# ElesionKyrie/Extreme-Video-Compression-With-Prediction-Using-Pre-trainded-Diffusion-Models-

Measured on AMD Instinct MI355X. Metric: decoded frames/sec (128x128x30) at q3, higher is better.
Workload: dtype f32

## Files before the change

extreme-video-compression-with-prediction-using-pre-trainded-diffusion-models-_amd/csrc/conv_small.hip:

```cpp
#include <hip/hip_runtime.h>
#include <stdint.h>
#include <stdio.h>
#include "../../include/evc_hip.h"
#include "split_mfma.h"

namespace {

struct SmallK {
    const float* src0; const float* src1; int C0, C1;
    const float* coef_a; const float* coef_s; const unsigned* in_bound;
    const char* w;
    const float* w_hdr;
    const float* bias; const float* res; float out_scale;
    float* out; float* stats;
    int H, HW, Co, CoPad, nchunk;
    int MT, NT, linear;
};

__device__ __forceinline__ float small_silu(float v) { return v * __builtin_amdgcn_rcpf(1.0f + __expf(-v)); }

template <bool AFFINE>
__device__ __forceinline__ float4 small_transform(float4 v, const float4& a, const float4& s, bool ok) {
    if (AFFINE) {
        v.x = small_silu(v.x * a.x + s.x); v.y = small_silu(v.y * a.y + s.y);
// ... 213 lines not shown
                if (t == 3) {
                    stage_store((it & 1) ^ 1);
                    __builtin_amdgcn_sched_barrier(0);
                }
            }
        }
        __syncthreads();
    }

    float* const red = reinterpret_cast<float*>(smem);
    if (g > 0) {
        float* o = red + (size_t)((g - 1) * NW + wv) * (TM * 16 * 64) + lane;
#pragma unroll
        for (int i = 0; i < TM; ++i)
#pragma unroll
            for (int r = 0; r < 16; ++r) o[(i * 16 + r) * 64] = acc[i][r];
    }
    __syncthreads();
    if (g > 0) return;
#pragma unroll 1
    for (int gg = 1; gg < G; ++gg) {
        const float* o = red + (size_t)((gg - 1) * NW + wv) * (TM * 16 * 64) + lane;
#pragma unroll
        for (int i = 0; i < TM; ++i)
#pragma unroll
            for (int r = 0; r < 16; ++r) acc[i][r] += o[(i * 16 + r) * 64];
    }
    if (p.res) {
        if (p.stats) small_epilogue<true, true>(p, acc, m0, n0, wm, wn, l31, half);
        else small_epilogue<true, false>(p, acc, m0, n0, wm, wn, l31, half);
    } else {
        if (p.stats) small_epilogue<false, true>(p, acc, m0, n0, wm, wn, l31, half);
        else small_epilogue<false, false>(p, acc, m0, n0, wm, wn, l31, half);
    }
}


struct SmallVariant { int W, wm, wn, g; };
constexpr SmallVariant SMALL_VARIANTS[4] = {
    {8, 1, 1, 8},
    {8, 1, 2, 4},
    {16, 2, 1, 4},
    {16, 2, 2, 2},
};

struct SmallLaunch {
    int variant;
    bool affine;
    dim3 grid;
    int threads;
    SmallK k;
};

int small_resolve(const evc_small_conv_args* a, SmallLaunch& p) {
    if (!a || !a->src0 || !a->w_packed || !a->out) return EVC_EINVAL;
    if (a->B <= 0 || a->H <= 0 || a->W <= 0 || a->C0 <= 0 || a->C1 < 0 || a->Co <= 0) return EVC_EINVAL;
    if ((a->C1 > 0) != (a->src1 != nullptr)) return EVC_EINVAL;
    if ((a->coef_a != nullptr) != (a->coef_s != nullptr)) return EVC_EINVAL;
    if (a->arith != EVC_ARITH_F16X3) return EVC_EUNSUPPORTED;
    if (a->KH != 3 || a->KW != 3) return EVC_EUNSUPPORTED;
    if (a->H != a->W || (a->H != 8 && a->H != 16)) return EVC_EUNSUPPORTED;
    if (a->invariant || a->x2_w_packed) return EVC_EUNSUPPORTED;
    if (a->act_out != EVC_ACT_NONE) return EVC_EUNSUPPORTED;
    if (a->coef_a ? a->act_in != EVC_ACT_SILU : a->act_in != EVC_ACT_NONE) return EVC_EUNSUPPORTED;
    if (a->C0 % 16 != 0 || a->C1 % 16 != 0 || a->Co % 32 != 0) return EVC_EUNSUPPORTED;
    const long long HW = (long long)a->H * a->W, M = HW * a->B, Ct = (long long)a->C0 + a->C1;
// ... 42 lines not shown
    SmallLaunch p;
    return small_resolve(a, p) == EVC_OK ? 1 : 0;
}

extern "C" int evc_small_conv_plan_query(const evc_small_conv_args* a, evc_small_conv_plan* out) {
    SmallLaunch p;
    const int rc = !out ? EVC_EINVAL : small_resolve(a, p);
    if (rc != EVC_OK) return rc;
    const SmallVariant& sv = SMALL_VARIANTS[p.variant - 1];
    small_kernel_name(p, out->kernel, (int)sizeof(out->kernel));
    out->variant = p.variant; out->tile_m = 64 * sv.wm; out->tile_n = 32 * sv.wn; out->groups = sv.g;
    out->chunks = p.k.nchunk; out->rounds = (p.k.nchunk + sv.g - 1) / sv.g; out->stats_runs = p.k.HW / 64;
    return EVC_OK;
}

extern "C" int evc_small_conv_f32(const evc_small_conv_args* a, void* stream) {
    SmallLaunch p;
    const int rc = small_resolve(a, p);
    if (rc != EVC_OK) return rc;
    SmallK& k = p.k;
    k.src0 = a->src0; k.src1 = a->src1; k.coef_a = a->coef_a; k.coef_s = a->coef_s; k.in_bound = a->in_bound;
    k.w_hdr = a->w_packed;
    k.w = reinterpret_cast<const char*>(a->w_packed) + F16_HDR_BYTES;
    k.bias = a->bias; k.res = a->res; k.out_scale = a->out_scale; k.out = a->out; k.stats = a->stats_out;
    hipStream_t st = (hipStream_t)stream;
    switch (p.variant) {
        case 1: small_launch<1, 1, 8>(p, st); break;
        case 2: small_launch<1, 2, 4>(p, st); break;
        case 3: small_launch<2, 1, 4>(p, st); break;
        default: small_launch<2, 2, 2>(p, st); break;
    }
    return hipGetLastError() == hipSuccess ? EVC_OK : EVC_ELAUNCH;
}
```

extreme-video-compression-with-prediction-using-pre-trainded-diffusion-models-_amd/lib.py:

```python
import ctypes
import math
import os
from ctypes import POINTER, c_char_p, c_double, c_float, c_int, c_int32, c_longlong, c_uint, c_uint8, c_ulonglong, c_void_p

import numpy as np
import torch

HERE = os.path.dirname(os.path.abspath(__file__))
HIP_SO = os.path.join(HERE, "lib", "libevc_hip.so")
if os.environ.get("EVC_HIP_SO"):
    HIP_SO = os.path.abspath(os.environ["EVC_HIP_SO"])
RANS_SO = os.path.join(HERE, "lib", "libevc_rans.so")

ACT_NONE, ACT_SILU, ACT_RELU = 0, 1, 2
ARITH_F32, ARITH_BF16X6, ARITH_F16X3 = 0, 1, 2
_ARITH_NAMES = {"f32": ARITH_F32, "bf16x6": ARITH_BF16X6, "f16x3": ARITH_F16X3}
_ARITH_DTYPES = {ARITH_F32: torch.float32, ARITH_BF16X6: torch.bfloat16, ARITH_F16X3: torch.float16}


def _arith_policy():
    name = os.environ.get("EVC_CONV_ARITH", "f16x3").lower()
    if name not in _ARITH_NAMES:
        raise ValueError(f"EVC_CONV_ARITH must be one of {sorted(_ARITH_NAMES)}, got {name!r}")
    return _ARITH_NAMES[name]
# ... 28 lines not shown
                ("x2_src0", c_void_p), ("x2_src1", c_void_p), ("x2_C0", c_int), ("x2_C1", c_int), ("x2_ld0", c_int),
                ("x2_ld1", c_int), ("x2_w_packed", c_void_p), ("x2_bound", c_void_p), ("invariant", c_int)]


class ConvPlan(ctypes.Structure):
    _fields_ = [("kernel", ctypes.c_char * 96), ("tile_m", c_int), ("tile_n", c_int), ("splits", c_int),
                ("steps_per_split", c_int), ("cut_chunk", c_int), ("tail_tiles", c_int), ("tail_splits", c_int),
                ("stats_runs", c_int), ("fused_1x1", c_int)]


class NinArgs(ctypes.Structure):
    _fields_ = [("x", c_void_p), ("x1", c_void_p), ("Ci", c_int), ("Co", c_int), ("coef_a", c_void_p), ("coef_s", c_void_p),
                ("in_bound", c_void_p), ("w_packed", c_void_p), ("arith", c_int), ("bias", c_void_p), ("res", c_void_p),
                ("out_scale", c_float), ("act_out", c_int), ("out", c_void_p), ("stats_out", c_void_p),
                ("B", c_int), ("H", c_int), ("W", c_int), ("tile", c_int)]


class NinPlan(ctypes.Structure):
    _fields_ = [("kernel", ctypes.c_char * 64), ("tile_m", c_int), ("tile_n", c_int), ("stages", c_int), ("stats_runs", c_int)]


class SmallConvArgs(ctypes.Structure):
    _fields_ = [("src0", c_void_p), ("src1", c_void_p), ("C0", c_int), ("C1", c_int),
                ("coef_a", c_void_p), ("coef_s", c_void_p), ("act_in", c_int), ("in_bound", c_void_p),
                ("w_packed", c_void_p), ("arith", c_int), ("bias", c_void_p), ("res", c_void_p),
                ("out_scale", c_float), ("act_out", c_int), ("out", c_void_p), ("stats_out", c_void_p),
                ("B", c_int), ("H", c_int), ("W", c_int), ("Co", c_int), ("KH", c_int), ("KW", c_int),
                ("x2_w_packed", c_void_p), ("invariant", c_int), ("variant", c_int)]


class SmallConvPlan(ctypes.Structure):
    _fields_ = [("kernel", ctypes.c_char * 64), ("variant", c_int), ("tile_m", c_int), ("tile_n", c_int), ("groups", c_int),
                ("chunks", c_int), ("rounds", c_int), ("stats_runs", c_int)]


class AttentionPlan(ctypes.Structure):
    _fields_ = [("kernel", ctypes.c_char * 64), ("waves", c_int), ("kparts", c_int), ("tiles_per_part", c_int),
                ("kv_planes", c_int), ("merge", c_int), ("short_seq", c_int),
                ("lds_bytes", c_longlong), ("parts_bytes", c_longlong), ("ws_bytes", c_longlong)]


HIP_SYMBOLS = {
    "evc_version": (c_char_p, []),
    "evc_arch": (c_char_p, []),
    "evc_device_ok": (c_int, []),
    "evc_clock_probe": (c_int, [c_void_p, c_int, c_void_p, c_void_p]),
    "evc_im2col_nchw_f32": (c_int, [c_void_p, c_void_p] + [c_int] * 9 + [c_void_p, c_void_p, c_void_p]),
    "evc_maxpool3s2_nhwc_f32": (c_int, [c_void_p, c_void_p, c_int, c_int, c_int, c_int, c_void_p]),
    "evc_lpips_layer_f32": (c_int, [c_void_p, c_void_p, c_void_p, c_void_p, c_int, c_int, c_int, c_int, c_void_p]),
    "evc_maxpool2d_nhwc_f32": (c_int, [c_void_p, c_void_p] + [c_int] * 7 + [c_void_p]),
    "evc_lpips_map_f32": (c_int, [c_void_p, c_void_p, c_void_p, c_void_p, c_int, c_int, c_int, c_void_p]),
    "evc_lpips_map_mean_f32": (c_int, [c_void_p, c_void_p, c_int, c_int, c_int, c_void_p]),
    "evc_lpips_upsample_add_f32": (c_int, [c_void_p, c_void_p] + [c_int] * 6 + [c_void_p]),
    "evc_i3d_stem_im2col_f32": (c_int, [c_void_p, c_void_p] + [c_int] * 17 + [c_void_p]),
    "evc_maxpool3d_same_nthwc_f32": (c_int, [c_void_p, c_void_p] + [c_int] * 11 + [c_void_p]),
    "evc_i3d_head_f32": (c_int, [c_void_p] * 4 + [c_int] * 6 + [c_void_p]),
    "evc_upfirdn2d_f32": (c_int, [c_void_p, c_void_p, POINTER(c_float)] + [c_int] * 13 + [c_void_p]),
    "evc_upfirdn2d_nhwc_f32": (c_int, [c_void_p, c_void_p, POINTER(c_float)] + [c_int] * 10 +
                               [c_void_p, c_void_p, c_int, c_void_p]),
    "evc_pack_nchw_to_nhwc_f32": (c_int, [c_void_p, c_int, c_void_p, c_int, c_void_p, c_int, c_int, c_int, c_int,
                                          c_void_p]),
    "evc_nhwc_to_nchw_f32": (c_int, [c_void_p, c_int, c_void_p, c_int, c_int, c_int, c_int, c_void_p]),
    "evc_chan_stats_f32": (c_int, [c_void_p, c_void_p, c_int, c_int, c_int, c_int, c_void_p]),
    "evc_gn_coeffs_f32": (c_int, [c_void_p, c_int, c_int, c_void_p, c_int, c_int, c_int, c_int, c_int, c_float,
                                  c_int, c_void_p, c_void_p, c_void_p, c_int, c_void_p, c_void_p, c_void_p,
                                  c_void_p]),
# ... 25 lines not shown
    "evc_conv5x5s2_phase_weights_f32": (c_int, [c_void_p, c_void_p, c_int, c_int, c_int, c_void_p]),
    "evc_depth_to_space2_f32": (c_int, [c_void_p, c_int, c_int, c_void_p, c_int, c_int, c_int, c_int, c_void_p]),
    "evc_space_to_depth2_f32": (c_int, [c_void_p, c_int, c_int, c_void_p, c_int, c_int, c_int, c_int, c_int, c_void_p]),
    "evc_deconv5x5s2_workspace_bytes": (c_longlong, [c_int, c_int, c_int, c_int]),
    "evc_deconv5x5s2_f32": (c_int, [c_void_p, c_void_p, c_int, c_void_p, c_void_p, c_void_p] + [c_int] * 6 + [c_void_p]),
    "evc_conv5x5s2_workspace_bytes": (c_longlong, [c_int, c_int, c_int, c_int]),
    "evc_conv5x5s2_f32": (c_int, [c_void_p, c_int, c_void_p, c_int, c_void_p, c_void_p, c_void_p] + [c_int] * 6 + [c_void_p]),
    "evc_gdn_workspace_bytes": (c_longlong, [c_int, c_int, c_int, c_int]),
    "evc_gdn_f32": (c_int, [c_void_p, c_void_p, c_int, c_void_p, c_void_p, c_void_p, c_int, c_int, c_int, c_int, c_int,
                            c_int, c_void_p]),
    "evc_affine_act_nhwc_f32": (c_int, [c_void_p, c_void_p, c_void_p, c_void_p, c_int, c_int, c_int, c_int, c_int,
                                        c_int, c_void_p]),
    "evc_conv_co_pad": (c_int, [c_int]),
    "evc_conv_packed_floats": (c_longlong, [c_int, c_int, c_int, c_int]),
    "evc_conv_pack_weights_f32": (c_int, [c_void_p, c_void_p, c_int, c_int, c_int, c_int, c_void_p]),
    "evc_conv_packed_bytes": (c_longlong, [c_int, c_int, c_int, c_int, c_int]),
    "evc_conv_pack_weights": (c_int, [c_void_p, c_void_p, c_int, c_int, c_int, c_int, c_int, c_void_p]),
    "evc_conv_set_option": (c_int, [c_char_p, c_int]),
    "evc_spade_act_nhwc_f32": (c_int, [c_void_p, c_void_p, c_void_p, c_void_p, c_int, c_void_p, c_void_p, c_int, c_void_p,
                                       c_void_p, c_int, c_void_p, c_int, c_int, c_int, c_int, c_int, c_void_p]),
    "evc_conv_choose_splits": (c_int, [POINTER(ConvArgs)]),
    "evc_conv_kernel_name": (c_int, [POINTER(ConvArgs), c_char_p, c_int]),
    "evc_conv_fused_1x1_supported": (c_int, [POINTER(ConvArgs)]),
    "evc_conv_stats_splits": (c_int, [POINTER(ConvArgs)]),
    "evc_conv_workspace_bytes": (c_longlong, [POINTER(ConvArgs)]),
    "evc_conv2d_nhwc_f32": (c_int, [POINTER(ConvArgs), c_void_p, c_void_p]),
    "evc_conv2d_nhwc_profiled_f32": (c_int, [POINTER(ConvArgs), c_void_p, c_void_p, c_void_p, c_void_p]),
    "evc_nin_gemm_supported": (c_int, [POINTER(NinArgs)]),
    "evc_nin_gemm_plan_query": (c_int, [POINTER(NinArgs), POINTER(NinPlan)]),
    "evc_nin_gemm_f32": (c_int, [POINTER(NinArgs), c_void_p]),
    "evc_small_conv_supported": (c_int, [POINTER(SmallConvArgs)]),
    "evc_small_conv_plan_query": (c_int, [POINTER(SmallConvArgs), POINTER(SmallConvPlan)]),
    "evc_small_conv_f32": (c_int, [POINTER(SmallConvArgs), c_void_p]),
    "evc_attention_f32": (c_int, [c_void_p, c_void_p, c_void_p, c_int, c_void_p, c_int, c_int, c_int, c_int, c_int,
                                  c_float, c_void_p]),
    "evc_attention_workspace_bytes": (c_longlong, [c_int, c_int, c_int, c_int]),
    "evc_attention_set_option": (c_int, [c_char_p, c_int]),
    "evc_attention_plan_query": (c_int, [c_int, c_int, c_int, c_int, c_int, c_int, c_int, POINTER(AttentionPlan)]),
    "evc_attention_ws_f32": (c_int, [c_void_p, c_void_p, c_void_p, c_int, c_void_p, c_int, c_int, c_int, c_int, c_int,
                                     c_float, c_void_p, c_void_p]),
    "evc_frame_group_norm_f32": (c_int, [c_void_p] * 4 + [c_int] * 5 + [c_float, c_void_p]),
    "evc_frame_attention_f32": (c_int, [c_void_p, c_int, c_void_p, c_int] + [c_int] * 5 + [c_float, c_void_p]),
    "evc_frame_mix_f32": (c_int, [c_void_p] * 4 + [c_int] * 3 + [c_longlong, c_void_p]),
    "evc_frame_taps_f32": (c_int, [c_void_p, c_void_p] + [c_int] * 4 + [c_void_p]),
    "evc_ddpm_step_f32": (c_int, [c_void_p, c_void_p, c_void_p, c_longlong] + [c_float] * 5 + [c_int, c_void_p]),
    "evc_ddim_step_f32": (c_int, [c_void_p, c_void_p, c_longlong] + [c_float] * 4 + [c_int, c_void_p]),
    "evc_axpy_f32": (c_int, [c_void_p, c_void_p, c_void_p, c_longlong, c_float, c_void_p]),
    "evc_pndm_transfer_f32": (c_int, [c_void_p, c_void_p, c_void_p, c_longlong, c_float, c_float, c_float, c_int,
                                      c_void_p]),
    "evc_lincomb4_f32": (c_int, [c_void_p] * 5 + [c_longlong] + [c_float] * 4 + [c_void_p]),
    "evc_scale_clamp_f32": (c_int, [c_void_p, c_void_p, c_longlong, c_float, c_float, c_int, c_float, c_float,
                                    c_void_p]),
    "evc_gate_residual_f32": (c_int, [c_void_p, c_void_p, c_void_p, c_void_p, c_longlong, c_void_p]),
    "evc_elic_gather_params_f32": (c_int, [c_void_p] + [c_int] * 8 + [c_void_p, c_int, c_void_p, c_void_p,
                                                                       c_void_p]),
    "evc_elic_scatter_symbols_f32": (c_int, [c_void_p, c_void_p, c_void_p] + [c_int] * 7 + [c_void_p]),
    "evc_elic_quantize_f32": (c_int, [c_void_p, c_int, c_int, c_void_p] + [c_int] * 5 + [c_void_p, c_void_p]),
    "evc_elic_rate_pass_f32": (c_int, [c_void_p] + [c_int] * 4 + [c_void_p] + [c_int] * 6 + [c_void_p, c_void_p, c_void_p]),
    "evc_bottleneck_rate_f32": (c_int, [c_void_p] + [c_int] * 5 + [c_void_p] * 5),
    "evc_noise_normal_f32": (c_int, [c_void_p, c_void_p, c_int, c_longlong, c_ulonglong, c_uint, c_int, c_void_p]),
    "evc_yuv420_to_rgb": (c_int, [c_void_p] + [c_longlong] * 6 + [c_int] * 5 + [c_void_p, c_int, c_void_p]),
    "evc_rgb_to_yuv420": (c_int, [c_void_p, c_void_p] + [c_longlong] * 6 + [c_int] * 4 + [c_void_p, c_void_p]),
    "evc_resample_h_u8": (c_int, [c_void_p, c_int, c_int, c_int, c_longlong, c_longlong, c_void_p, c_void_p, c_int, c_int, c_void_p,
                                  c_void_p]),
    "evc_resample_v_u8": (c_int, [c_void_p, c_int, c_int, c_int, c_longlong, c_longlong, c_void_p, c_void_p, c_int, c_int, c_void_p,
                                  c_void_p]),
# ... 757 lines not shown
                chunks=out.chunks, rounds=out.rounds, stats_runs=out.stats_runs)


def small_conv(src0, w_packed, Co, bias=None, src1=None, coef=None, act_in=ACT_NONE, res=None, out_scale=1.0, in_bound=None,
               want_stats=False, out=None, variant=0):
    L = hip_lib()
    B, H, W, C0 = src0.shape
    C1 = 0 if src1 is None else src1.shape[-1]
    for t, c in ((src0, C0), (src1, C1), (res, Co)):
        assert t is None or (t.is_contiguous() and t.dtype == torch.float32 and t.shape == (B, H, W, c))
    if out is None:
        out = torch.empty((B, H, W, Co), device=src0.device, dtype=torch.float32)
    assert out.is_contiguous() and out.shape == (B, H, W, Co)
    ca, cs = coef if coef is not None else (None, None)
    assert ca is None or (ca.shape == (B, C0 + C1) and cs.shape == (B, C0 + C1) and ca.is_contiguous() and cs.is_contiguous())
    a = SmallConvArgs(src0=ptr(src0), src1=ptr(src1), C0=C0, C1=C1, coef_a=ptr(ca), coef_s=ptr(cs), act_in=act_in,
                      in_bound=_word(in_bound), w_packed=ptr(w_packed), arith=packed_arith(w_packed), bias=ptr(bias),
                      res=ptr(res), out_scale=float(out_scale), act_out=ACT_NONE, out=ptr(out), B=B, H=H, W=W, Co=Co, KH=3, KW=3,
                      variant=variant)
    plan = SmallConvPlan()
    _check(L.evc_small_conv_plan_query(ctypes.byref(a), ctypes.byref(plan)), "evc_small_conv_plan_query")
    stats = None
    if want_stats:
        stats = torch.empty((B, plan.stats_runs, Co, 2), device=src0.device, dtype=torch.float32)
        a.stats_out = ptr(stats)
    _check(L.evc_small_conv_f32(ctypes.byref(a), stream_ptr()), "evc_small_conv_f32")
    if SMALL_CONV_PROFILE is not None:
        SMALL_CONV_PROFILE.append(dict(kernel=plan.kernel.decode(), tile=(plan.tile_m, plan.tile_n), groups=plan.groups,
                                       shape=(B, H, W, C0 + C1, Co), C1=C1, coef=coef is not None, bound=in_bound is not None,
                                       res=res is not None, stats=bool(want_stats)))
    return (out, stats) if want_stats else out


def attention_set_option(name, value):
    if hip_lib(require_device=False).evc_attention_set_option(name.encode(), int(value)) != 0:
        raise EvcKernelError(f"unknown attention option {name!r}")


ATTN_PROFILE = None


def attention_plan(B, heads, N, D, with_bounds=False, have_ws=None, invariant=False):
    L = hip_lib(require_device=False)
    if have_ws is None:
        nbytes = (L.evc_attention_invariant_workspace_bytes if invariant else L.evc_attention_workspace_bytes)(B, heads, N, D)
        have_ws = nbytes > 0
    out = AttentionPlan()
    _check(L.evc_attention_plan_query(B, heads, N, D, int(bool(with_bounds)), int(bool(have_ws)), int(bool(invariant)),
                                      ctypes.byref(out)), "evc_attention_plan_query")
    return dict(kernel=out.kernel.decode(), waves=out.waves, kparts=out.kparts, tiles_per_part=out.tiles_per_part,
                kv_planes=bool(out.kv_planes), merge=bool(out.merge), short_seq=bool(out.short_seq),
                lds_bytes=out.lds_bytes, parts_bytes=out.parts_bytes, ws_bytes=out.ws_bytes)


def attention(qkv, C, heads, out=None, bounds=None, invariant=False, ws=None):
    L = hip_lib()
    B, N, ld = qkv.shape
    D = C // heads
    inv = bool(invariant)
    if out is None:
        out = torch.empty((B, N, C), device=qkv.device, dtype=torch.float32)
    ld_out = out.shape[-1]
    assert out.is_contiguous() and tuple(out.shape[:2]) == (B, N) and ld_out >= C
    base = qkv.data_ptr()
    nbytes = (L.evc_attention_invariant_workspace_bytes if inv else L.evc_attention_workspace_bytes)(B, heads, N, D)
    if ws is None:
# ... 542 lines not shown
```

extreme-video-compression-with-prediction-using-pre-trainded-diffusion-models-_amd/scorenet.py:

```python
import math
from types import SimpleNamespace

import numpy as np
import torch

from . import lib as L

FIR_K = np.outer([1, 3, 3, 1], [1, 3, 3, 1]).astype(np.float32)
FIR_K /= FIR_K.sum()
INV_SQRT2 = float(np.float32(1.0) / np.sqrt(np.float32(2.0)))


def num_groups(ch):
    g = min(ch // 4, 32)
    while ch % g != 0:
        g -= 1
    return g


def dims_from_config(config):
    m, d = config.model, config.data
    return SimpleNamespace(ngf=m.ngf, ch_mult=list(m.ch_mult), num_res_blocks=m.num_res_blocks,
                           attn_resolutions=list(m.attn_resolutions), n_head_channels=m.n_head_channels,
                           image_size=d.image_size, channels=d.channels, num_frames=d.num_frames,
# ... 170 lines not shown
        self.embed_dim = self._embed_dim()
        self.program = self._build_program()
        if self.SPADE:
            self.program[2]["cin"] = self.d.channels * self.d.num_frames
        self._wsrc = {}
        self._load(state_dict, prefix + "unet.all_modules.")
        self.sites = range_sites(self.program, self.cond_emb) if self.RANGE_SITES else []
        self.site_words = L.site_word_arena(len(self.sites), self.device)
        self._demoted = set()
        self._attn_f32 = set()
        self._unfused = set()
        self._site_of = {}
        self._set_site_args()
        self.demote_seconds = 0.0
        self._rows = {}
        self._row_tensors = {}
        self._table = torch.zeros((256, self.ss_total), device=self.device, dtype=torch.float32)
        self._n_rows = 0
        self.use_graphs = use_graphs
        self._graphs = {}
        self._f16_raw = L.bounded_arith() == L.ARITH_F16X3
        import os
        self.overlap_skip = os.environ.get("EVC_OVERLAP_SKIP", "1") != "0"
        self.fuse_skip = self._f16_raw and os.environ.get("EVC_FUSE_SKIP", "1") != "0"
        self._side_streams = {}
        self._bounds_by_stream = {}
        self._bounds = None
        self._bound_next = 0
        self._bound_batch = 1
        if demote:
            self.demote(demote)

    def _conv(self, *a, **kw):
        return self._conv_routed(*a, **kw) if self.small_conv else L.conv2d_nhwc(*a, invariant=self.batch_invariant, **kw)

    def _act(self, t, stats=None):
        return _Act(t, stats, invariant=self.batch_invariant)

    def _gn(self, *a, **kw):
        return L.gn_coeffs(*a, invariant=self.batch_invariant, **kw)

    def _mbound(self, *a, **kw):
        return L.moments_bound(*a, invariant=self.batch_invariant, **kw)

    def _attention(self, *a, **kw):
        return L.attention(*a, invariant=self.batch_invariant, **kw)

    def _fuse_ok(self, *a, **kw):
        return L.conv_fused_1x1_supported(*a, invariant=self.batch_invariant, **kw)

    def invariant_view(self):
        import copy
        if self.batch_invariant:
            return self
        if self.SPADE or self.ARCH != "unetmore" or self.noise_in_cond:
            raise NotImplementedError("batch_invariant is built for the concat-conditioned score network (ScoreNet) only")
        if self._demoted:
            raise ValueError("batch-invariant mode does not combine with demoted sites (range recovery)")
        v = copy.copy(self)
        v.batch_invariant = True
        v.taps = None
        v._rows, v._row_tensors = {}, {}
        v._table = torch.zeros_like(self._table)
        v._n_rows = 0
        v._graphs, v._side_streams, v._bounds_by_stream = {}, {}, {}
        v._bounds, v._bound_next = None, 0
        return v
# ... 267 lines not shown

    def _attn(self, i, m, x):
        e = self.w[i]
        B, H, W, C = x.t.shape
        hd = self.d.n_head_channels
        heads = 1 if C < hd else C // hd
        coef = self._gn([x.stats()], H * W, num_groups(C), 1e-6, mode=1, gamma=e["gamma"], beta=e["beta"],
                           site=self._site("attn_norm", i))
        qkvb = self._bound_slot(3)
        if qkvb is None:
            obound = None
            qkv = self._proj(x.t, e["wqkv"], 3 * C, e["bqkv"], coef=coef)
        else:
            qkv, qst = self._proj(x.t, e["wqkv"], 3 * C, e["bqkv"], coef=coef, want_stats=True)
            self._mbound(qst, 0, C, qkvb, site=self._site("attn_qkv", i))
            obound = _f16_only(e["wo"], qkvb.view(B, 3)[:, 2].contiguous() if self.batch_invariant else qkvb[2:3])
        o = self._attention(qkv.view(B, H * W, 3 * C), C, heads, bounds=None if i in self._attn_f32 else qkvb)
        return self._act(*self._proj(o.view(B, H, W, C), e["wo"], C, e["bo"], res=x.t, out_scale=INV_SQRT2, want_stats=True,
                                     in_bound=obound))

    nin_gemm = True

    def _proj(self, x, w, Co, bias, coef=None, res=None, out_scale=1.0, want_stats=False, in_bound=None):
        B, H, W, Ci = x.shape
        plain = not self.batch_invariant and not self.SPADE and self.ARCH == "unetmore"
        if self.nin_gemm and plain and L.packed_arith(w) == L.ARITH_F16X3 and \
                L.nin_gemm_supported(B, H, W, Ci, Co, coef=coef is not None, bound=in_bound is not None):
            return L.nin_gemm(x, w, Co, bias=bias, coef=coef, res=res, out_scale=out_scale, in_bound=in_bound,
                              want_stats=want_stats)
        return self._conv(x, w, Co, 1, 1, bias=bias, coef=coef, res=res, out_scale=out_scale, want_stats=want_stats,
                          in_bound=in_bound)

    small_conv = True

    def _conv_routed(self, src0, w, Co, KH, KW, src1=None, x2=None, out=None, act_out=L.ACT_NONE, splits=0, **kw):
        plain = not self.batch_invariant and not self.SPADE and self.ARCH == "unetmore"
        dense = torch.is_tensor(src0) and (src1 is None or torch.is_tensor(src1))
        if plain and dense and KH == 3 and KW == 3 and x2 is None and out is None and act_out == L.ACT_NONE and not splits \
                and L.packed_arith(w) == L.ARITH_F16X3:
            B, H, W, C0 = src0.shape
            if L.small_conv_supported(B, H, W, C0, 0 if src1 is None else src1.shape[-1], Co, coef=kw.get("coef") is not None,
                                      act_in=kw.get("act_in", L.ACT_NONE), bound=kw.get("in_bound") is not None):
                return L.small_conv(src0, w, Co, src1=src1, **kw)
        return L.conv2d_nhwc(src0, w, Co, KH, KW, src1=src1, x2=x2, out=out, act_out=act_out, splits=splits,
                             invariant=self.batch_invariant, **kw)

    @torch.no_grad()
    def forward_rows(self, x, rows, cond=None):
        if self.batch_invariant and self._demoted:
            raise ValueError("batch-invariant mode does not combine with demoted sites (range recovery)")
        return self._forward_rows(x, rows, cond)

    def _forward_rows(self, x, rows, cond=None):
        d = self.d
        prog = self.program
        B, _, H, W = x.shape
        self._bound_batch = B if self.batch_invariant else 1
        nb = 256 * self._bound_batch
        if self._f16_raw:
            if torch.cuda.is_current_stream_capturing():
                self._bounds = torch.empty(nb, device=self.device, dtype=torch.int32)
            else:
                key = torch.cuda.current_stream().cuda_stream
                self._bounds = self._bounds_by_stream.get(key)
                if self._bounds is None or self._bounds.numel() != nb:
                    self._bounds = self._bounds_by_stream[key] = torch.empty(nb, device=self.device, dtype=torch.int32)
            self._bounds.zero_()
            self._bound_next = 0
        taps = getattr(self, "taps", None)

        def tap(idx, act):
            if taps is not None:
                taps[idx] = act.t[..., :prog[idx].get("cout", prog[idx].get("ch"))].permute(0, 3, 1, 2).contiguous()
            return act
        i = 2
        m = prog[i]
# ... 112 lines not shown
```

include/evc_hip.h:

```cpp
#ifndef EVC_HIP_H
#define EVC_HIP_H

#ifdef __cplusplus
extern "C" {
#endif

#define EVC_OK 0
#define EVC_EINVAL (-1)
#define EVC_EUNSUPPORTED (-2)
#define EVC_ELAUNCH (-3)

#define EVC_ACT_NONE 0
#define EVC_ACT_SILU 1
#define EVC_ACT_RELU 2

#define EVC_ARITH_F32 0
#define EVC_ARITH_BF16X6 1
#define EVC_ARITH_F16X3 2

const char* evc_version(void);
const char* evc_arch(void);
int evc_device_ok(void);

int evc_clock_probe(unsigned long long* out2, int spin_us, const unsigned* stop, void* stream);
// ... 104 lines not shown
    float* out; float* stats_out;
    int B; int H; int W;
    int tile;
} evc_nin_args;
typedef struct {
    char kernel[64];
    int tile_m, tile_n, stages, stats_runs;
} evc_nin_plan;
int evc_nin_gemm_supported(const evc_nin_args* a);
int evc_nin_gemm_plan_query(const evc_nin_args* a, evc_nin_plan* out);
int evc_nin_gemm_f32(const evc_nin_args* a, void* stream);

typedef struct {
    const float* src0; const float* src1; int C0; int C1;
    const float* coef_a; const float* coef_s; int act_in;
    const unsigned* in_bound;
    const float* w_packed; int arith;
    const float* bias; const float* res;
    float out_scale; int act_out;
    float* out; float* stats_out;
    int B; int H; int W; int Co; int KH; int KW;
    const float* x2_w_packed;
    int invariant;
    int variant;
} evc_small_conv_args;
typedef struct {
    char kernel[64];
    int variant, tile_m, tile_n, groups, chunks, rounds, stats_runs;
} evc_small_conv_plan;
int evc_small_conv_supported(const evc_small_conv_args* a);
int evc_small_conv_plan_query(const evc_small_conv_args* a, evc_small_conv_plan* out);
int evc_small_conv_f32(const evc_small_conv_args* a, void* stream);

int evc_attention_f32(const float* q, const float* k, const float* v, int ld_qkv, float* out, int ld_out, int B,
                      int heads, int N, int D, float scale, void* stream);
long long evc_attention_workspace_bytes(int B, int heads, int N, int D);
int evc_attention_set_option(const char* name, int value);
int evc_attention_ws_f32(const float* q, const float* k, const float* v, int ld_qkv, float* out, int ld_out, int B,
                         int heads, int N, int D, float scale, float* ws, void* stream);

int evc_attention_f16x3_f32(const float* q, const float* k, const float* v, int ld_qkv, float* out, int ld_out, int B,
                            int heads, int N, int D, float scale, const unsigned* bounds, float* ws, void* stream);

typedef struct {
    char kernel[64];
    int waves, kparts, tiles_per_part, kv_planes, merge, short_seq;
    long long lds_bytes, parts_bytes, ws_bytes;
} evc_attention_plan;
int evc_attention_plan_query(int B, int heads, int N, int D, int with_bounds, int have_ws, int invariant,
                             evc_attention_plan* out);

int evc_frame_group_norm_f32(const float* x, float* y, const float* gamma, const float* beta, int B, int N, int HW, int C,
                             int groups, float eps, void* stream);
int evc_frame_attention_f32(const float* qkv, int ld_qkv, float* out, int ld_out, int B, int N, int HW, int C, int heads,
                            float scale, void* stream);
int evc_frame_mix_f32(const float* x, float* y, const float* w, const float* bias, int B, int N, int M, long long inner,
                      void* stream);

int evc_frame_taps_f32(const float* x, float* y, int B, int N, int HW, int C, void* stream);

int evc_ddpm_step_f32(float* x, const float* e, const float* noise, long long n, float k1, float k2, float c1,
                      float c2, float sigma, int clip, void* stream);
int evc_ddim_step_f32(float* x, const float* e, long long n, float k1, float k2, float c1, float c2, int clip,
                      void* stream);
int evc_axpy_f32(const float* x, const float* e, float* y, long long n, float alpha, void* stream);
int evc_pndm_transfer_f32(const float* x, const float* e, float* y, long long n, float d, float cx, float ce,
// ... 106 lines not shown
```

Baseline: 39.55.

## Add 16x16 3x3 conv kernel with 64x96 tiles and split-K wave groups

Adds a dedicated kernel for 3x3 convolutions at 16x16 resolution with Co=576. Each block computes a 64x96 output tile, with four wave groups splitting the input-channel chunks. The kernel stages the input halo in LDS with double buffering, software-pipelines weight loads across the nine taps, and reduces partial sums through shared memory. The scorenet router uses it when the existing small-conv kernel does not apply. The aim is to replace the generic conv path for these layers with better weight reuse and wave occupancy. The cost is more code to maintain and a narrow support envelope.

```diff
diff --git a/extreme-video-compression-with-prediction-using-pre-trainded-diffusion-models-_amd/csrc/conv_small.hip b/extreme-video-compression-with-prediction-using-pre-trainded-diffusion-models-_amd/csrc/conv_small.hip
--- a/extreme-video-compression-with-prediction-using-pre-trainded-diffusion-models-_amd/csrc/conv_small.hip
+++ b/extreme-video-compression-with-prediction-using-pre-trainded-diffusion-models-_amd/csrc/conv_small.hip
@@ -269,6 +269,213 @@
     } else {
         if (p.stats) small_epilogue<false, true>(p, acc, m0, n0, wm, wn, l31, half);
         else small_epilogue<false, false>(p, acc, m0, n0, wm, wn, l31, half);
+    }
+}
+
+struct TnGeom {
+    static constexpr int W = 16, R = 4, SW = W + 2, SPX = (R + 2) * SW;
+    static constexpr int HPL = SPX * 16, APL = SPX * 32, IMG = 2 * APL, GRP = 2 * IMG;
+};
+
+template <int TN, int G, bool AFFINE>
+__global__ __launch_bounds__(64 * G) void conv_small_tn_kernel(SmallK p) {
+    typedef Split<2> SP;
+    typedef SP::vec vec;
+    typedef TnGeom GE;
+    constexpr int TM = 2, BM = 64, BN = 32 * TN, RB = 32, KC = 16;
+    constexpr int W = GE::W, R = GE::R, SW = GE::SW, HPL = GE::HPL, APL = GE::APL, IMG = GE::IMG, GRP = GE::GRP;
+    constexpr int PIX = (R + 2) * W;
+    constexpr int NU = 2 * PIX / 64;
+    static_assert(2 * PIX == NU * 64, "the staging units divide over one wave");
+    static_assert((G - 1) * TN * 16 * 64 * 4 <= G * GRP, "one batch of the reduction fits the staging images");
+    __shared__ __attribute__((aligned(16))) char smem[G * GRP];
+
+    int nt, mt;
+    {
+        const int id = blockIdx.x;
+        const int T = p.NT * p.MT, tile = p.linear ? id : (id & 7) * ((T + 7) >> 3) + (id >> 3);
+        if (tile >= T) return;
+        nt = tile / p.MT; mt = tile - nt * p.MT;
+    }
+    const int m0 = mt * BM, n0 = nt * BN;
+
+    const int lane = threadIdx.x & 63;
+    const int g = __builtin_amdgcn_readfirstlane(threadIdx.x >> 6);
+    const int l31 = lane & 31, half = lane >> 5;
+    char* const As = smem + g * GRP;
+
+    const int per = (p.nchunk + G - 1) / G;
+    const int c_begin = min(p.nchunk, g * per), c_end = min(p.nchunk, c_begin + per);
+    const bool busy = c_begin < c_end;
+
+    const int bimg = m0 / p.HW;
+    const int y0 = (m0 - bimg * p.HW) / W;
+    const int Ct = p.C0 + p.C1;
+
+    const int kh = lane & 1;
+    unsigned goff0[NU], goff1[NU];
+    int slds[NU];
+    bool sval[NU];
+#pragma unroll
+    for (int k = 0; k < NU; ++k) {
+        const int pp = (lane + 64 * k) >> 1;
+        const int sr = pp / W, x = pp - sr * W;
+        const int y = y0 + sr - 1;
+        sval[k] = y >= 0 && y < p.H;
+        const unsigned pix = (unsigned)((bimg * p.H + (sval[k] ? y : 0)) * W + x);
+        goff0[k] = (pix * (unsigned)p.C0 + 8u * kh) * 4u;
+        goff1[k] = (pix * (unsigned)p.C1 + 8u * kh) * 4u;
+        slds[k] = kh * HPL + (sr * SW + x + 1) * 16;
+    }
+    int abase[TM];
+#pragma unroll
+    for (int i = 0; i < TM; ++i) {
+        const int ml = i * 32 + l31;
+        const int r = ml / W, x = ml - r * W;
+        abase[i] = half * HPL + (r * SW + x) * 16;
+    }
+    const unsigned planeB = (unsigned)p.CoPad * RB;
+    const unsigned slab = 2u * planeB;
+    const unsigned w_tap = (unsigned)p.nchunk * slab;
+    const char* const wlane = p.w + (unsigned)(n0 + l31) * RB + 16u * (unsigned)(half ^ ((l31 >> 3) & 1));
+    auto load_b = [&](vec (&bb)[TN][2], int c, int t) {
+        const char* wt = wlane + ((unsigned)t * w_tap + (unsigned)c * slab);
+#pragma unroll
+        for (int j = 0; j < TN; ++j) {
+            bb[j][0] = *reinterpret_cast<const vec*>(wt + j * 32 * RB);
+            bb[j][1] = *reinterpret_cast<const vec*>(wt + j * 32 * RB + planeB);
+        }
+    };
+
+    const float xscale = F16_ACT_SCALE * (p.in_bound ? bound_scale(p.in_bound[0]) : 1.0f);
+    float4 xr[NU][2], ca[2], cs[2];
+    auto stage_load = [&](int c) {
+        const int cc = c * KC;
+        const bool first = cc < p.C0;
+        const char* src = reinterpret_cast<const char*>(first ? p.src0 : p.src1);
+        const unsigned cb = (unsigned)(first ? cc : cc - p.C0) * 4u;
+#pragma unroll
+        for (int k = 0; k < NU; ++k) {
+            const unsigned o = (first ? goff0[k] : goff1[k]) + cb;
+            xr[k][0] = *reinterpret_cast<const float4*>(src + o);
+            xr[k][1] = *reinterpret_cast<const float4*>(src + o + 16);
+        }
+        if (AFFINE) {
+            const size_t co = (size_t)bimg * Ct + cc + 8 * kh;
+            ca[0] = *reinterpret_cast<const float4*>(p.coef_a + co);
+            ca[1] = *reinterpret_cast<const float4*>(p.coef_a + co + 4);
+            cs[0] = *reinterpret_cast<const float4*>(p.coef_s + co);
+            cs[1] = *reinterpret_cast<const float4*>(p.coef_s + co + 4);
+        }
+    };
+    auto stage_store = [&](int buf) {
+#pragma unroll
+        for (int k = 0; k < NU; ++k) {
+            vec pl[2];
+            SP::split(small_transform<AFFINE>(xr[k][0], ca[0], cs[0], sval[k]),
+                      small_transform<AFFINE>(xr[k][1], ca[1], cs[1], sval[k]), xscale, pl);
+            char* A = As + buf * IMG + slds[k];
+            *reinterpret_cast<vec*>(A) = pl[0];
+            *reinterpret_cast<vec*>(A + APL) = pl[1];
+        }
+    };
+    vec a[2][TM][2];
+    auto read_a = [&](vec (&aa)[TM][2], const char* img, int t) {
+        const int toff = ((t / 3) * SW + (t % 3)) * 16;
+#pragma unroll
+        for (int i = 0; i < TM; ++i) {
+            aa[i][0] = *reinterpret_cast<const vec*>(img + abase[i] + toff);
+            aa[i][1] = *reinterpret_cast<const vec*>(img + APL + abase[i] + toff);
+        }
+    };
+
+    f32x16 acc[TN][TM];
+#pragma unroll
+    for (int j = 0; j < TN; ++j)
+#pragma unroll
+        for (int i = 0; i < TM; ++i)
+#pragma unroll
+            for (int r = 0; r < 16; ++r) acc[j][i][r] = 0.f;
+
+    vec b[3][TN][2];
+    if (busy) {
+        stage_load(c_begin);
+        load_b(b[0], c_begin, 0);
+        load_b(b[1], c_begin, 1);
+    }
+    for (int u = lane; u < 2 * (R + 2) * 8; u += 64) {
+        const int ph = u & 3, side = (u >> 2) & 1, q = u >> 3;
+        const int buf = q / (R + 2), row = q - buf * (R + 2);
+        const int spx = row * SW + (side ? W + 1 : 0);
+        *reinterpret_cast<float4*>(As + buf * IMG + (ph >> 1) * APL + (ph & 1) * HPL + spx * 16) = make_float4(0.f, 0.f, 0.f, 0.f);
+    }
+    if (busy) stage_store(0);
+    __syncthreads();
+
+    for (int it = 0; it < per; ++it) {
+        const int c = c_begin + it;
+        if (c < c_end) {
+            const int cn = min(c + 1, c_end - 1);
+            stage_load(cn);
+            const char* img = As + (it & 1) * IMG;
+            read_a(a[0], img, 0);
+            __builtin_amdgcn_sched_barrier(0);
+#pragma unroll
+            for (int t = 0; t < 9; ++t) {
+                if (t < 8) read_a(a[(t + 1) & 1], img, t + 1);
+                if (t < 7) load_b(b[(t + 2) % 3], c, t + 2);
+                else load_b(b[(t + 2) % 3], cn, t - 7);
+                __builtin_amdgcn_sched_barrier(0);
+#pragma unroll
+                for (int q = 0; q < SP::NTERM; ++q)
+#pragma unroll
+                    for (int j = 0; j < TN; ++j)
+#pragma unroll
+                        for (int i = 0; i < TM; ++i)
+                            acc[j][i] = SP::mfma(a[t & 1][i][SP::qa(q)], b[t % 3][j][SP::qb(q)], acc[j][i]);
+                __builtin_amdgcn_sched_barrier(0);
+                if (t == 3) {
+                    stage_store((it & 1) ^ 1);
+                    __builtin_amdgcn_sched_barrier(0);
+                }
+            }
+        }
+        __syncthreads();
+    }
+
+    float* const red = reinterpret_cast<float*>(smem);
+#pragma unroll
+    for (int i = 0; i < TM; ++i) {
+        if (i) __syncthreads();
+        if (g > 0) {
+            float* o = red + (size_t)(g - 1) * (TN * 16 * 64) + lane;
+#pragma unroll
+            for (int j = 0; j < TN; ++j)
+#pragma unroll
+                for (int r = 0; r < 16; ++r) o[(j * 16 + r) * 64] = acc[j][i][r];
+        }
+        __syncthreads();
+        if (g == 0) {
+#pragma unroll 1
+            for (int gg = 1; gg < G; ++gg) {
+                const float* o = red + (size_t)(gg - 1) * (TN * 16 * 64) + lane;
+#pragma unroll
+                for (int j = 0; j < TN; ++j)
+#pragma unroll
+                    for (int r = 0; r < 16; ++r) acc[j][i][r] += o[(j * 16 + r) * 64];
+            }
+        }
+    }
+    if (g > 0) return;
+#pragma unroll
+    for (int j = 0; j < TN; ++j) {
+        if (p.res) {
+            if (p.stats) small_epilogue<true, true>(p, acc[j], m0, n0 + 32 * j, 0, 0, l31, half);
+            else small_epilogue<true, false>(p, acc[j], m0, n0 + 32 * j, 0, 0, l31, half);
+        } else {
+            if (p.stats) small_epilogue<false, true>(p, acc[j], m0, n0 + 32 * j, 0, 0, l31, half);
+            else small_epilogue<false, false>(p, acc[j], m0, n0 + 32 * j, 0, 0, l31, half);
+        }
     }
 }
 
@@ -377,3 +584,83 @@
     }
     return hipGetLastError() == hipSuccess ? EVC_OK : EVC_ELAUNCH;
 }
+
+
+namespace {
+
+constexpr int TN_G = 4;
+
+struct TnLaunch {
+    int variant;
+    bool affine;
+    dim3 grid;
+    SmallK k;
+};
+
+int tn_resolve(const evc_small96_conv_args* a, TnLaunch& p) {
+    if (!a || !a->src0 || !a->w_packed || !a->out) return EVC_EINVAL;
+    if (a->B <= 0 || a->H <= 0 || a->W <= 0 || a->C0 <= 0 || a->C1 < 0 || a->Co <= 0) return EVC_EINVAL;
+    if ((a->C1 > 0) != (a->src1 != nullptr)) return EVC_EINVAL;
+    if ((a->coef_a != nullptr) != (a->coef_s != nullptr)) return EVC_EINVAL;
+    if (a->arith != EVC_ARITH_F16X3) return EVC_EUNSUPPORTED;
+    if (a->KH != 3 || a->KW != 3) return EVC_EUNSUPPORTED;
+    if (a->H != 16 || a->W != 16) return EVC_EUNSUPPORTED;
+    if (a->invariant || a->x2_w_packed) return EVC_EUNSUPPORTED;
+    if (a->act_out != EVC_ACT_NONE) return EVC_EUNSUPPORTED;
+    if (a->coef_a ? a->act_in != EVC_ACT_SILU : a->act_in != EVC_ACT_NONE) return EVC_EUNSUPPORTED;
+    if (a->C0 % 16 != 0 || a->C1 % 16 != 0 || a->Co % 96 != 0) return EVC_EUNSUPPORTED;
+    const long long HW = 256, M = HW * a->B, Ct = (long long)a->C0 + a->C1;
+    if (M * (a->C0 > a->C1 ? a->C0 : a->C1) * 4 >= (1LL << 32) || M * a->Co >= (1LL << 31)) return EVC_EUNSUPPORTED;
+    if (9 * Ct * 2 * evc_conv_co_pad(a->Co) * 2 >= (1LL << 32)) return EVC_EUNSUPPORTED;
+    const int v = a->variant & 15;
+    if ((a->variant & ~31) != 0 || v > 1) return EVC_EUNSUPPORTED;
+    p.variant = 1;
+    if (!v) {
+        const long long T = (long long)(a->Co / 96) * 4 * a->B;
+        if (a->Co != 576 || Ct < 384 || T < 216 || T > 256) return EVC_EUNSUPPORTED;
+    }
+    p.affine = a->coef_a != nullptr;
+    SmallK& k = p.k;
+    k.C0 = a->C0; k.C1 = a->C1; k.H = 16; k.HW = (int)HW; k.Co = a->Co; k.CoPad = evc_conv_co_pad(a->Co);
+    k.nchunk = (int)(Ct / 16);
+    k.MT = (int)(M / 64); k.NT = a->Co / 96; k.linear = (a->variant >> 4) & 1;
+    p.grid = dim3((unsigned)(k.linear ? k.NT * k.MT : (k.NT * k.MT + 7) / 8 * 8));
+    return EVC_OK;
+}
+
+void tn_launch(const TnLaunch& p, hipStream_t st) {
+    if (p.affine) hipLaunchKernelGGL((conv_small_tn_kernel<3, TN_G, true>), p.grid, dim3(64 * TN_G), 0, st, p.k);
+    else hipLaunchKernelGGL((conv_small_tn_kernel<3, TN_G, false>), p.grid, dim3(64 * TN_G), 0, st, p.k);
+}
+
+}
+
+extern "C" int evc_small96_conv_supported(const evc_small96_conv_args* a) {
+    TnLaunch p;
+    return tn_resolve(a, p) == EVC_OK ? 1 : 0;
+}
+
+extern "C" int evc_small96_conv_plan_query(const evc_small96_conv_args* a, evc_small96_conv_plan* out) {
+    TnLaunch p;
+    const int rc = !out ? EVC_EINVAL : tn_resolve(a, p);
+    if (rc != EVC_OK) return rc;
+    const int g = TN_G;
+    snprintf(out->kernel, sizeof(out->kernel), "conv_small_tn_kernel<3, %d, %s>", g, p.affine ? "true" : "false");
+    out->variant = p.variant; out->tile_m = 64; out->tile_n = 96; out->groups = g;
+    out->chunks = p.k.nchunk; out->rounds = (p.k.nchunk + g - 1) / g; out->stats_runs = p.k.HW / 64;
+    return EVC_OK;
+}
+
+extern "C" int evc_small96_conv_f32(const evc_small96_conv_args* a, void* stream) {
+    TnLaunch p;
+    const int rc = tn_resolve(a, p);
+    if (rc != EVC_OK) return rc;
+    SmallK& k = p.k;
+    k.src0 = a->src0; k.src1 = a->src1; k.coef_a = a->coef_a; k.coef_s = a->coef_s; k.in_bound = a->in_bound;
+    k.w_hdr = a->w_packed;
+    k.w = reinterpret_cast<const char*>(a->w_packed) + F16_HDR_BYTES;
+    k.bias = a->bias; k.res = a->res; k.out_scale = a->out_scale; k.out = a->out; k.stats = a->stats_out;
+    hipStream_t st = (hipStream_t)stream;
+    tn_launch(p, st);
+    return hipGetLastError() == hipSuccess ? EVC_OK : EVC_ELAUNCH;
+}
diff --git a/extreme-video-compression-with-prediction-using-pre-trainded-diffusion-models-_amd/lib.py b/extreme-video-compression-with-prediction-using-pre-trainded-diffusion-models-_amd/lib.py
--- a/extreme-video-compression-with-prediction-using-pre-trainded-diffusion-models-_amd/lib.py
+++ b/extreme-video-compression-with-prediction-using-pre-trainded-diffusion-models-_amd/lib.py
@@ -84,6 +84,14 @@
 class SmallConvPlan(ctypes.Structure):
     _fields_ = [("kernel", ctypes.c_char * 64), ("variant", c_int), ("tile_m", c_int), ("tile_n", c_int), ("groups", c_int),
                 ("chunks", c_int), ("rounds", c_int), ("stats_runs", c_int)]
+
+
+class Small96ConvArgs(ctypes.Structure):
+    _fields_ = list(SmallConvArgs._fields_)
+
+
+class Small96ConvPlan(ctypes.Structure):
+    _fields_ = list(SmallConvPlan._fields_)
 
 
 class AttentionPlan(ctypes.Structure):
@@ -175,6 +183,9 @@
     "evc_small_conv_supported": (c_int, [POINTER(SmallConvArgs)]),
     "evc_small_conv_plan_query": (c_int, [POINTER(SmallConvArgs), POINTER(SmallConvPlan)]),
     "evc_small_conv_f32": (c_int, [POINTER(SmallConvArgs), c_void_p]),
+    "evc_small96_conv_supported": (c_int, [POINTER(Small96ConvArgs)]),
+    "evc_small96_conv_plan_query": (c_int, [POINTER(Small96ConvArgs), POINTER(Small96ConvPlan)]),
+    "evc_small96_conv_f32": (c_int, [POINTER(Small96ConvArgs), c_void_p]),
     "evc_attention_f32": (c_int, [c_void_p, c_void_p, c_void_p, c_int, c_void_p, c_int, c_int, c_int, c_int, c_int,
                                   c_float, c_void_p]),
     "evc_attention_workspace_bytes": (c_longlong, [c_int, c_int, c_int, c_int]),
@@ -998,6 +1009,63 @@
     return (out, stats) if want_stats else out
 
 
+SMALL96_CONV_PROFILE = None
+
+
+def small96_conv_query_args(B, H, W, C0, C1, Co, K=3, arith=ARITH_F16X3, coef=False, act_in=None, bound=False,
+                            act_out=ACT_NONE, x2=False, invariant=False, variant=0):
+    d = c_void_p(16)
+    act_in = (ACT_SILU if coef else ACT_NONE) if act_in is None else act_in
+    return Small96ConvArgs(src0=d, src1=d if C1 else None, C0=C0, C1=C1, coef_a=d if coef else None,
+                           coef_s=d if coef else None, act_in=act_in, in_bound=d if bound else None, w_packed=d, arith=arith,
+                           out_scale=1.0, act_out=act_out, out=d, B=B, H=H, W=W, Co=Co, KH=K, KW=K,
+                           x2_w_packed=d if x2 else None, invariant=int(bool(invariant)), variant=variant)
+
+
+def small96_conv_supported(B, H, W, C0, C1, Co, **kw):
+    a = small96_conv_query_args(B, H, W, C0, C1, Co, **kw)
+    return bool(hip_lib(require_device=False).evc_small96_conv_supported(ctypes.byref(a)))
+
+
+def small96_conv_plan(B, H, W, C0, C1, Co, **kw):
+    out = Small96ConvPlan()
+    a = small96_conv_query_args(B, H, W, C0, C1, Co, **kw)
+    _check(hip_lib(require_device=False).evc_small96_conv_plan_query(ctypes.byref(a), ctypes.byref(out)),
+           "evc_small96_conv_plan_query")
+    return dict(kernel=out.kernel.decode(), variant=out.variant, tile=(out.tile_m, out.tile_n), groups=out.groups,
+                chunks=out.chunks, rounds=out.rounds, stats_runs=out.stats_runs)
+
+
+def small96_conv(src0, w_packed, Co, bias=None, src1=None, coef=None, act_in=ACT_NONE, res=None, out_scale=1.0, in_bound=None,
+                 want_stats=False, out=None, variant=0):
+    L = hip_lib()
+    B, H, W, C0 = src0.shape
+    C1 = 0 if src1 is None else src1.shape[-1]
+    for t, c in ((src0, C0), (src1, C1), (res, Co)):
+        assert t is None or (t.is_contiguous() and t.dtype == torch.float32 and t.shape == (B, H, W, c))
+    if out is None:
+        out = torch.empty((B, H, W, Co), device=src0.device, dtype=torch.float32)
+    assert out.is_contiguous() and out.shape == (B, H, W, Co)
+    ca, cs = coef if coef is not None else (None, None)
+    assert ca is None or (ca.shape == (B, C0 + C1) and cs.shape == (B, C0 + C1) and ca.is_contiguous() and cs.is_contiguous())
+    a = Small96ConvArgs(src0=ptr(src0), src1=ptr(src1), C0=C0, C1=C1, coef_a=ptr(ca), coef_s=ptr(cs), act_in=act_in,
+                        in_bound=_word(in_bound), w_packed=ptr(w_packed), arith=packed_arith(w_packed), bias=ptr(bias),
+                        res=ptr(res), out_scale=float(out_scale), act_out=ACT_NONE, out=ptr(out), B=B, H=H, W=W, Co=Co, KH=3,
+                        KW=3, variant=variant)
+    plan = Small96ConvPlan()
+    _check(L.evc_small96_conv_plan_query(ctypes.byref(a), ctypes.byref(plan)), "evc_small96_conv_plan_query")
+    stats = None
+    if want_stats:
+        stats = torch.empty((B, plan.stats_runs, Co, 2), device=src0.device, dtype=torch.float32)
+        a.stats_out = ptr(stats)
+    _check(L.evc_small96_conv_f32(ctypes.byref(a), stream_ptr()), "evc_small96_conv_f32")
+    if SMALL96_CONV_PROFILE is not None:
+        SMALL96_CONV_PROFILE.append(dict(kernel=plan.kernel.decode(), tile=(plan.tile_m, plan.tile_n), groups=plan.groups,
+                                         shape=(B, H, W, C0 + C1, Co), C1=C1, coef=coef is not None,
+                                         bound=in_bound is not None, res=res is not None, stats=bool(want_stats)))
+    return (out, stats) if want_stats else out
+
+
 def attention_set_option(name, value):
     if hip_lib(require_device=False).evc_attention_set_option(name.encode(), int(value)) != 0:
         raise EvcKernelError(f"unknown attention option {name!r}")
diff --git a/extreme-video-compression-with-prediction-using-pre-trainded-diffusion-models-_amd/scorenet.py b/extreme-video-compression-with-prediction-using-pre-trainded-diffusion-models-_amd/scorenet.py
--- a/extreme-video-compression-with-prediction-using-pre-trainded-diffusion-models-_amd/scorenet.py
+++ b/extreme-video-compression-with-prediction-using-pre-trainded-diffusion-models-_amd/scorenet.py
@@ -226,7 +226,7 @@
             self.demote(demote)
 
     def _conv(self, *a, **kw):
-        return self._conv_routed(*a, **kw) if self.small_conv else L.conv2d_nhwc(*a, invariant=self.batch_invariant, **kw)
+        return self._conv_routed(*a, **kw) if self._routing else L.conv2d_nhwc(*a, invariant=self.batch_invariant, **kw)
 
     def _act(self, t, stats=None):
         return _Act(t, stats, invariant=self.batch_invariant)
@@ -560,6 +560,8 @@
                           in_bound=in_bound)
 
     small_conv = True
+    small96_conv = True
+    _routing = property(lambda self: self.small_conv or self.small96_conv)
 
     def _conv_routed(self, src0, w, Co, KH, KW, src1=None, x2=None, out=None, act_out=L.ACT_NONE, splits=0, **kw):
         plain = not self.batch_invariant and not self.SPADE and self.ARCH == "unetmore"
@@ -567,9 +569,12 @@
         if plain and dense and KH == 3 and KW == 3 and x2 is None and out is None and act_out == L.ACT_NONE and not splits \
                 and L.packed_arith(w) == L.ARITH_F16X3:
             B, H, W, C0 = src0.shape
-            if L.small_conv_supported(B, H, W, C0, 0 if src1 is None else src1.shape[-1], Co, coef=kw.get("coef") is not None,
-                                      act_in=kw.get("act_in", L.ACT_NONE), bound=kw.get("in_bound") is not None):
+            q = dict(coef=kw.get("coef") is not None, act_in=kw.get("act_in", L.ACT_NONE), bound=kw.get("in_bound") is not None)
+            C1 = 0 if src1 is None else src1.shape[-1]
+            if self.small_conv and L.small_conv_supported(B, H, W, C0, C1, Co, **q):
                 return L.small_conv(src0, w, Co, src1=src1, **kw)
+            if self.small96_conv and L.small96_conv_supported(B, H, W, C0, C1, Co, **q):
+                return L.small96_conv(src0, w, Co, src1=src1, **kw)
         return L.conv2d_nhwc(src0, w, Co, KH, KW, src1=src1, x2=x2, out=out, act_out=act_out, splits=splits,
                              invariant=self.batch_invariant, **kw)
 
diff --git a/include/evc_hip.h b/include/evc_hip.h
--- a/include/evc_hip.h
+++ b/include/evc_hip.h
@@ -160,6 +160,27 @@
 int evc_small_conv_plan_query(const evc_small_conv_args* a, evc_small_conv_plan* out);
 int evc_small_conv_f32(const evc_small_conv_args* a, void* stream);
 
+typedef struct {
+    const float* src0; const float* src1; int C0; int C1;
+    const float* coef_a; const float* coef_s; int act_in;
+    const unsigned* in_bound;
+    const float* w_packed; int arith;
+    const float* bias; const float* res;
+    float out_scale; int act_out;
+    float* out; float* stats_out;
+    int B; int H; int W; int Co; int KH; int KW;
+    const float* x2_w_packed;
+    int invariant;
+    int variant;
+} evc_small96_conv_args;
+typedef struct {
+    char kernel[64];
+    int variant, tile_m, tile_n, groups, chunks, rounds, stats_runs;
+} evc_small96_conv_plan;
+int evc_small96_conv_supported(const evc_small96_conv_args* a);
+int evc_small96_conv_plan_query(const evc_small96_conv_args* a, evc_small96_conv_plan* out);
+int evc_small96_conv_f32(const evc_small96_conv_args* a, void* stream);
+
 int evc_attention_f32(const float* q, const float* k, const float* v, int ld_qkv, float* out, int ld_out, int B,
                       int heads, int N, int D, float scale, void* stream);
 long long evc_attention_workspace_bytes(int B, int heads, int N, int D);
```

Measured after the change: 39.79, median of 6. About the same (+0.6%).
